# toandaominh1997/EfficientDet.Pytorch

Hardware: AMD Instinct MI355X
Metric: images/sec EfficientDet-D0 512px fwd+bwd (higher is better)
Workload: dtype f32_hf16x3_bwd_bf16x3

## Files before the change

### efficientdet/pytorch_amd/_lib.py

```python
import ctypes as C
import os

import torch

HERE = os.path.dirname(os.path.abspath(__file__))
LIB_PATH = os.environ.get('EFFDET_HIP_LIB') or os.path.join(os.path.dirname(os.path.abspath(__file__)), 'libeffdet_hip.so')
MAX_SEG = 5
MAX_CONV_SEG = 10
ABI_VERSION = 11
F32, BF16, F32_BF16X3, F32_SPLIT = 0, 1, 2, 3
F32_HSPLIT = 4
ACT_NONE, ACT_RELU, ACT_SWISH, ACT_SIGMOID = 0, 1, 2, 3
RES_NONE, RES_ADD, RES_RELU_MASK, RES_SWISH_GRAD = 0, 1, 2, 3
TUNE_IGEMM_BIG, TUNE_IGEMM_BIG_MIN_M, TUNE_SPLIT_PERS, TUNE_IGEMM_KORD, TUNE_SPLIT_KORD = 0, 1, 2, 3, 4
TUNE_ROWSLAB = 5
TUNE_SHORT_TILE = 7

_ERR = {-1: 'EFFDET_EINVAL', -2: 'EFFDET_ELAUNCH', -3: 'EFFDET_EUNSUPPORTED'}


class Seg(C.Structure):
    _fields_ = [('H', C.c_int), ('W', C.c_int), ('Ho', C.c_int), ('Wo', C.c_int),
                ('in_off', C.c_longlong), ('in_bstride', C.c_longlong),
                ('out_off', C.c_longlong), ('out_bstride', C.c_longlong)]


class ConvDesc(C.Structure):
    _fields_ = [('x', C.c_void_p), ('w', C.c_void_p), ('y', C.c_void_p), ('z', C.c_void_p), ('res', C.c_void_p),
                ('scale', C.c_void_p), ('shift', C.c_void_p), ('rowscale', C.c_void_p),
                ('bc_scale', C.c_void_p), ('bc_shift', C.c_void_p),
                ('dtype', C.c_int), ('out_f32', C.c_int),
# ... 78 lines not shown

class QualityLoss(C.Structure):
    _fields_ = [('kind', C.c_int), ('beta', C.c_float), ('alpha', C.c_float), ('gamma', C.c_float)]


TAL_MAX_TOPK = 16


class Tal(C.Structure):
    _fields_ = [('topk', C.c_int), ('alpha', C.c_float), ('beta', C.c_float), ('aligned_target', C.c_int)]


class ConvPlanInfo(C.Structure):
    _fields_ = [(n, C.c_int) for n in ('id', 'form', 'persistent', 'tile_m', 'tile_n', 'stages', 'threads', 'mtiles', 'ntiles', 'grid',
                                       'ksteps', 'kord', 'lds_bytes', 'm32')] + [('reserved', C.c_int * 2)]


class WgradPlanInfo(C.Structure):
    _fields_ = [(n, C.c_int) for n in ('path', 'splits', 'nfast', 'mchunk', 'ntiles', 'jtiles', 'stage_pixels', 'allr', 'thin_ns', 'gate',
                                       'nseg')] + [('first', C.c_int * MAX_SEG), ('count', C.c_int * MAX_SEG), ('reserved', C.c_int * 3)]


WBF_MAX_VIEWS, WBF_MAX_IN = 8, 4096


class Wbf(C.Structure):
    _fields_ = [(n, C.c_void_p * WBF_MAX_VIEWS) for n in ('score', 'label', 'boxes', 'count')] + \
               [('A', C.c_longlong * WBF_MAX_VIEWS)] + [(n, C.c_float * WBF_MAX_VIEWS) for n in ('weight', 'width', 'mul')] + \
               [('flip', C.c_int * WBF_MAX_VIEWS)] + [(n, C.c_int) for n in ('V', 'B', 'top_n', 'conf_type')] + \
               [('iou_thr', C.c_float), ('skip_thr', C.c_float)] + \
# ... 206 lines not shown
WGRAD_PAIR_SIGNATURES = {
    'effdet_conv2d_wgrad_pair': 'i:pppqps',
}
OPT_GROUPS_SIGNATURES = {
    'effdet_opt_step_groups': 'i:iippppppppppiiipppfiipps',
}
GATE_OPERAND_SIGNATURES = {
    'effdet_conv2d_gated': 'i:ppis',
    'effdet_conv2d_gated_plan_info': 'i:ppip',
    'effdet_conv2d_wgrad_gated': 'i:ppipqs',
    'effdet_conv2d_wgrad_gated_kernel': 'i:ppi',
}
WGRAD_PLAN_SIGNATURES = {
    'effdet_conv2d_wgrad_plan_info': 'i:pp',
}
RESAMPLE_SIGNATURES = {
    'effdet_resample_images': 'i:ps',
}
SLICES_SIGNATURES = {
    'effdet_slice_images': 'i:ps',
    'effdet_slice_merge_workspace_bytes': 'q:iii',
    'effdet_slice_merge': 'i:ppqs',
}
OP_POINT_SIGNATURES = {
    'effdet_op_curves_workspace_bytes': 'q:q',
    'effdet_op_curves': 'i:ppqpipipqppppppps',
    'effdet_confusion_match': 'i:ppppiiiifdps',
}
OP_MAX_THRESHOLDS = 4096
TRACK_SIGNATURES = {
# ... 23 lines not shown
        if not os.path.exists(LIB_PATH):
            raise RuntimeError(
                'libeffdet_hip.so is missing (%s). Build it with `python -m efficientdet.pytorch_amd.build` '
                '(or __graft_entry__.build()). There is no CPU fallback for this path.' % LIB_PATH)
        cand = C.CDLL(LIB_PATH)
        got = int(cand.effdet_abi_version()) if hasattr(cand, 'effdet_abi_version') else 0
        if got != ABI_VERSION:
            raise RuntimeError('%s has ABI generation %d, this binding needs %d: rebuild it (`python -m efficientdet.pytorch_amd.build`)'
                               % (LIB_PATH, got, ABI_VERSION))
        _lib = cand
        for name, sig in list(SIGNATURES.items()) + list(ADDED_SIGNATURES.items()) + list(EMA_SIGNATURES.items()) + \
                list(PLAN_SIGNATURES.items()) + list(LIVE_SIGNATURES.items()) + list(BOX_LOSS_SIGNATURES.items()) + \
                list(LOSS_OPTS_SIGNATURES.items()) + list(ATSS_SIGNATURES.items()) + list(CONV_PLAN_SIGNATURES.items()) + \
                list(WBF_SIGNATURES.items()) + list(NEEDED_SIGNATURES.items()) + list(MOSAIC_SIGNATURES.items()) + \
                list(WGRAD_PAIR_SIGNATURES.items()) + list(OPT_GROUPS_SIGNATURES.items()) + list(GATE_OPERAND_SIGNATURES.items()) + \
                list(WGRAD_PLAN_SIGNATURES.items()) + list(AFFINE_SIGNATURES.items()) + list(RESAMPLE_SIGNATURES.items()) + \
                list(UNIT_LISTS_SIGNATURES.items()) + list(SLICES_SIGNATURES.items()) + list(QUALITY_LOSS_SIGNATURES.items()) + \
                list(TAL_SIGNATURES.items()) + list(OP_POINT_SIGNATURES.items()) + list(TRACK_SIGNATURES.items()) + \
                list(ASSIGN_SIGNATURES.items()):
            f = getattr(_lib, name, None)
            if f is not None:
                f.restype, f.argtypes = _CTYPE[sig[0]], [_CTYPE[c] for c in sig[2:]]
    return _lib


def require(*names):
    L = lib()
    missing = [n for n in names if not hasattr(L, n)]
    if missing:
        raise RuntimeError('%s does not export %s: it predates this binding, rebuild it (`python -m efficientdet.pytorch_amd.build`)'
                           % (LIB_PATH, ', '.join(missing)))
# ... 28 lines not shown
```

### efficientdet/pytorch_amd/csrc/common.h

```cpp
#pragma once
#include <hip/hip_runtime.h>
#include <stdint.h>
#include "../../../include/effdet_hip.h"

typedef uint16_t bf16_t;
typedef float f32x4 __attribute__((ext_vector_type(4)));
typedef __bf16 bf16x8 __attribute__((ext_vector_type(8)));

#define EFFDET_CHECK_LAUNCH()                                 \
  do {                                                        \
    hipError_t e_ = hipGetLastError();                        \
    if (e_ != hipSuccess) return EFFDET_ELAUNCH;              \
  } while (0)

#define EFFDET_SET_MAX_LDS(kernel, bytes)                                                                           \
  do {                                                                                                              \
    static unsigned long long done_ = 0ull;                                                                         \
    int dev_ = 0;                                                                                                   \
    (void)hipGetDevice(&dev_);                                                                                      \
    const unsigned long long bit_ = 1ull << (dev_ & 63);                                                            \
    if (!(done_ & bit_)) {                                                                                          \
      (void)hipFuncSetAttribute((const void*)(kernel), hipFuncAttributeMaxDynamicSharedMemorySize, (int)(bytes));  \
      done_ |= bit_;                                                                                                \
    }                                                                                                               \
// ... 184 lines not shown
  return f32x4{__uint_as_float(v[0]), __uint_as_float(v[1]), __uint_as_float(v[2]), __uint_as_float(v[3])};
}
typedef unsigned u32x2_t __attribute__((ext_vector_type(2)));
template <> __device__ __forceinline__ f32x4 srd_load4<bf16_t>(__amdgpu_buffer_rsrc_t r, unsigned byte_off) {
  const u32x2_t u = __builtin_amdgcn_raw_buffer_load_b64(r, (int)byte_off, 0, 0);
  return f32x4{__uint_as_float(u[0] << 16), __uint_as_float(u[0] & 0xffff0000u), __uint_as_float(u[1] << 16),
               __uint_as_float(u[1] & 0xffff0000u)};
}

__device__ __forceinline__ int xcd_remap(int bid, int nwg) {
  const int q = nwg >> 3, r = nwg & 7;
  const int xcd = bid & 7, idx = bid >> 3;
  const int base = (xcd < r) ? xcd * (q + 1) : r * (q + 1) + (xcd - r) * q;
  return base + idx;
}
```

### efficientdet/pytorch_amd/csrc/conv_igemm.hip

```cpp
#include "common.h"
#include "../../../include/effdet_live_tiles.h"
#include "../../../include/effdet_needed_tiles.h"
#include "../../../include/effdet_unit_lists.h"
#include "../../../include/effdet_conv_plan.h"
#include "../../../include/effdet_gate_operand.h"
#include <stdlib.h>

#ifndef EFFDET_IGEMM_BIG_DEFAULT
#define EFFDET_IGEMM_BIG_DEFAULT 1
#endif

namespace {

struct SegD {
  int H, W, Ho, Wo, M, tile_start;
  long long in_off, in_bs, out_off, out_bs;
  unsigned x_bytes;
  long long w_off;
  long long sh_off;
};

struct ConvK {
  const void* x; const void* w; void* y; void* z; const void* res;
  const float* scale; const float* shift; const float* rowscale;
// ... 1205 lines not shown
}

struct ConvPlan {
  int id;
  ConvK k;
  int (*launch)(const ConvPlan&, hipStream_t);
  unsigned grid;
  size_t lds;
  int pw_G, pw_NPS, pw_ppw;
  int form, pers;
  int tile_m, tile_n, stages, threads, m32;
  int ksteps;
  int gate;
};

static int g_tuning[EFFDET_TUNE_COUNT] = {-1, 16384, -1, 1, -1, -1, 0 , 1};
static bool rowslab_on() {
  if (g_tuning[EFFDET_TUNE_ROWSLAB] < 0) g_tuning[EFFDET_TUNE_ROWSLAB] = getenv("EFFDET_ROWSLAB") ? atoi(getenv("EFFDET_ROWSLAB")) : 1;
  return g_tuning[EFFDET_TUNE_ROWSLAB] != 0;
}

template <typename T, int BN, int WAVES_N, int NWAVES, int SPLIT, int NS, int M32, int GATE, int BM>
int launch_igemm(const ConvPlan& c, hipStream_t st) {
  if (c.lds > 48 * 1024) EFFDET_SET_MAX_LDS((conv_igemm_kernel<T, BN, WAVES_N, NWAVES, SPLIT, NS, M32, GATE, BM>), c.lds);
  hipLaunchKernelGGL((conv_igemm_kernel<T, BN, WAVES_N, NWAVES, SPLIT, NS, M32, GATE, BM>), dim3(c.grid), dim3(NWAVES * 64), c.lds, st, c.k);
  EFFDET_CHECK_LAUNCH();
  return EFFDET_OK;
}
template <typename T, int BN, int WAVES_N, int NWAVES, int SPLIT = 0, int NS = 2, int M32 = 0, int GATE = 0, int BM = BM128>
int use_igemm(ConvPlan& c, int id) {
  if constexpr (BM != BM128) {
// ... 103 lines not shown
    }
    if (bt == 0) return use_igemm<T, 128, 2, 8, SPLIT, 4, 0, GATE>(c, id);
    if (bt == 1) return use_igemm<T, 64, 1, 4, SPLIT, 4, 0, GATE>(c, id);
  }
  switch (bt) {
    case 0: return use_igemm<T, 128, 2, 8, SPLIT, 2, 0, GATE>(c, id);
    case 1: return use_igemm<T, 64, 1, 4, SPLIT, 2, 0, GATE>(c, id);
    case 2: return use_igemm<T, 32, 1, 4, SPLIT, 2, 0, GATE>(c, id);
    default: return use_igemm<T, 16, 1, 4, SPLIT, 2, 0, GATE>(c, id);
  }
}

}

extern "C" int effdet_tuning_set(int key, int value) {
  if (key < 0 || key >= EFFDET_TUNE_COUNT || key == EFFDET_TUNE_ROWSLAB + 1) return EFFDET_EINVAL;
  (void)big_variant();
  const int old = g_tuning[key];
  g_tuning[key] = value;
  return old;
}

static int plan_conv(const effdet_conv_t* p, ConvPlan& c, const float* a_gate = nullptr, int a_act = EFFDET_ACT_NONE) {
  ConvK& k = c.k;
  c.gate = 0;
  if (!p || !p->x || !p->w || !p->y) return EFFDET_EINVAL;
  if (p->nseg < 1 || p->nseg > EFFDET_MAX_CONV_SEG) return EFFDET_EINVAL;
  if (p->dtype != EFFDET_F32 && p->dtype != EFFDET_BF16 && p->dtype != EFFDET_F32_BF16X3 && p->dtype != EFFDET_F32_SPLIT && p->dtype != EFFDET_F32_HSPLIT) return EFFDET_EINVAL;
  const int ce = p->dtype == EFFDET_BF16 ? 8 : 4;
  if (p->Cin % ce || p->ldx % ce || p->KH < 1 || p->KW < 1 || p->stride < 1) return EFFDET_EUNSUPPORTED;
  if (p->res_mode != EFFDET_RES_NONE && !p->res) return EFFDET_EINVAL;
  const bool hfmt = p->dtype == EFFDET_F32_HSPLIT;
  const bool splitfmt = p->dtype == EFFDET_F32_SPLIT || hfmt;
  if (hfmt && (p->res_mode != EFFDET_RES_NONE || p->scale || p->bc_scale || p->rowscale || p->w_image_stride || (p->KH * p->KW * p->Cin) % 32)) return EFFDET_EUNSUPPORTED;
  if (splitfmt) {
    if (p->Cin % 32 || p->ldx % 32 || p->z) return EFFDET_EUNSUPPORTED;
// ... 224 lines not shown
```

### efficientdet/pytorch_amd/csrc/conv_wgrad.hip

```cpp
#include "common.h"
#include "../../../include/effdet_gate_operand.h"
#include "../../../include/effdet_live_tiles.h"
#include "../../../include/effdet_wgrad_pair.h"
#include "../../../include/effdet_wgrad_plan.h"
#include <stdlib.h>

#ifndef EFFDET_WGRAD_TR_WAVES
#define EFFDET_WGRAD_TR_WAVES 8
#endif

namespace {

struct WSeg {
  int H, W, Ho, Wo, M, split_start;
  long long in_off, in_bs, out_off, out_bs;
  unsigned x_bytes, dz_bytes;
  int step0;
};
struct WgradK {
  const void* x; const void* dz; float* dw; float* dbias; float* slab;
  float* dbp;
  int Cin, Cout, KW, stride, pad_t, pad_l;
  int ldx, lddz;
  int B;
  int Kc, cpt;
  int K;
  int mchunk;
  int nseg, ntiles, jtiles, vec_a;
  const unsigned char* live32;
  const float* a_gate;
  int gate_hw;
  WSeg seg[EFFDET_MAX_SEG];
};

template <typename T> struct WMma;
template <> struct WMma<bf16_t> {
  static __device__ __forceinline__ void run(const uint4& a, const uint4& b, f32x4& c) {
    c = __builtin_amdgcn_mfma_f32_16x16x32_bf16(__builtin_bit_cast(bf16x8, a), __builtin_bit_cast(bf16x8, b), c, 0, 0, 0);
  }
  static __device__ __forceinline__ uint4 ones() { return make_uint4(0x3f803f80u, 0x3f803f80u, 0x3f803f80u, 0x3f803f80u); }
};
template <> struct WMma<float> {
  static __device__ __forceinline__ void run(const uint4& a, const uint4& b, f32x4& c) {
// ... 582 lines not shown
  const int prob = idx < nf ? q.first : q.first ^ 1;
  const int l = idx < nf ? f0 + idx : eighth((int)gridDim.x, xcd) - f0 + (idx - nf);
  int split, tile;
  if (LIVEB && prob == 1) { tile = l / q.splits[1]; split = q.splits[1] - 1 - (l - tile * q.splits[1]); }
  else { split = l / tiles; tile = l - split * tiles; }
  const int nt = tile % q.k.ntiles, jt = tile / q.k.ntiles;
  int si = 0;
#pragma unroll
  for (int s = 1; s < EFFDET_MAX_SEG; ++s)
    if (s < q.nseg[prob] && split >= q.seg[prob][s].split_start) si = s;
  const WSeg sg = q.seg[prob][si];
  if (LIVEB && prob == 1) wgrad_split_block<ALLR, 1>(q.k, sg, q.x[1], q.dz[1], q.slab[1], q.dbp[1], q.live32, nt, jt, split);
  else wgrad_split_block<ALLR, 0>(q.k, sg, q.x[prob], q.dz[prob], q.slab[prob], q.dbp[prob], nullptr, nt, jt, split);
}

template <int NW, int X3 = 0, int GATE = 0>
__global__ __launch_bounds__(NW * 64, (GATE && X3) ? 2 : 1) void conv_wgrad_f32dma_kernel(const WgradK p) {
  constexpr int WJ = NW / 2;
  constexpr int WTJ = 128 / WJ, JB = WTJ / 16;
  constexpr int BKM = 32;
  constexpr unsigned OPB = 16384, BUFB = 2 * OPB;
  constexpr int PPW = 16 / NW;

  extern __shared__ __attribute__((aligned(16))) uint4 smem[];
  const int tid = threadIdx.x, lane = tid & 63;
  const int wave = __builtin_amdgcn_readfirstlane(tid >> 6);
  const int wn0 = (wave / WJ) * 64, wj0 = (wave % WJ) * WTJ;
  const int logical = xcd_remap(blockIdx.x, gridDim.x);
  const int nt = logical % p.ntiles, jt = (logical / p.ntiles) % p.jtiles, split = logical / (p.ntiles * p.jtiles);
  int si = 0;
#pragma unroll
  for (int s = 1; s < EFFDET_MAX_SEG; ++s)
    if (s < p.nseg && split >= p.seg[s].split_start) si = s;
  const WSeg sg = p.seg[si];
  const int m_begin = (split - sg.split_start) * p.mchunk;
  const int m_end = min(sg.M, m_begin + p.mchunk);
  const int nsteps = (m_end - m_begin + BKM - 1) / BKM;
// ... 58 lines not shown
  float gb[JB];
  if constexpr (GATE) {
    const float* grow = p.a_gate + (long long)(m_begin / p.gate_hw) * p.K;
#pragma unroll
    for (int b = 0; b < JB; ++b) { const int j = jt * 128 + wj0 + JB * c15 + b; gb[b] = j < p.K ? grow[j] : 0.f; }
  }
  auto gate1 = [&](float v, int b) -> float {
    if constexpr (GATE == 2) v = swishf_(v);
    v *= gb[b];
    asm volatile("" : "+v"(v));
    return v;
  };

  if (nsteps > 0) {
    stage(0);
    if constexpr (X3) {
      typedef float f32x2l __attribute__((ext_vector_type(2)));
      auto split8 = [](const float (&v)[8], uint4& hi, uint4& lo) {
        unsigned h[4], l[4];
#pragma unroll
        for (int i = 0; i < 4; ++i) {
          h[i] = pack2bf(v[2 * i], v[2 * i + 1]);
          l[i] = pack2bf(v[2 * i] - __uint_as_float(h[i] << 16), v[2 * i + 1] - __uint_as_float(h[i] & 0xffff0000u));
        }
        hi = make_uint4(h[0], h[1], h[2], h[3]); lo = make_uint4(l[0], l[1], l[2], l[3]);
      };
      auto mm = [](const uint4& a, const uint4& b, f32x4& c) {
        c = __builtin_amdgcn_mfma_f32_16x16x32_bf16(__builtin_bit_cast(bf16x8, a), __builtin_bit_cast(bf16x8, b), c, 0, 0, 0);
      };
      const uint4 ones = make_uint4(0x3f803f80u, 0x3f803f80u, 0x3f803f80u, 0x3f803f80u);
      uint4 ah[4], al[4], bh[JB], bl[JB];
      bool have = false;
      auto mma_stage = [&]() {
#pragma unroll
        for (int t = 0; t < 3; ++t)
#pragma unroll
          for (int a = 0; a < 4; ++a)
#pragma unroll
            for (int b = 0; b < JB; ++b) mm(t == 0 ? al[a] : ah[a], t == 1 ? bl[b] : bh[b], acc[a][b]);
        if (want_bias) {
#pragma unroll
          for (int a = 0; a < 4; ++a) { mm(al[a], ones, bsum[a]); mm(ah[a], ones, bsum[a]); }
        }
      };
      for (int kt = 0; kt < nsteps; ++kt) {
        const unsigned cur = (unsigned)(kt & 1) * BUFB;
        dma_wait_all();
        __syncthreads();
        if (kt + 1 < nsteps) stage((kt & 1) ^ 1);
        f32x4 ra[8]; float rb[8][JB];
#pragma unroll
        for (int e = 0; e < 8; ++e) {
          ra[e] = *(const f32x4 __attribute__((address_space(3)))*)(size_t)(a_addr + cur + (unsigned)e * 2048u);
          if constexpr (JB == 4) {
            const f32x4 t = *(const f32x4 __attribute__((address_space(3)))*)(size_t)(b_addr + cur + (unsigned)e * 2048u);
#pragma unroll
            for (int b = 0; b < JB; ++b) rb[e][b] = t[b];
          } else {
            const f32x2l t = *(const f32x2l __attribute__((address_space(3)))*)(size_t)(b_addr + cur + (unsigned)e * 2048u);
            rb[e][0] = t[0]; rb[e][1] = t[1];
          }
        }
        __builtin_amdgcn_sched_barrier(0);
        if (have) mma_stage();
// ... 6 lines not shown
#pragma unroll
        for (int a = 0; a < 4; ++a) {
          const float v[8] = {ra[0][a], ra[1][a], ra[2][a], ra[3][a], ra[4][a], ra[5][a], ra[6][a], ra[7][a]};
          split8(v, ah[a], al[a]);
        }
#pragma unroll
        for (int b = 0; b < JB; ++b) {
          const float v[8] = {rb[0][b], rb[1][b], rb[2][b], rb[3][b], rb[4][b], rb[5][b], rb[6][b], rb[7][b]};
          split8(v, bh[b], bl[b]);
        }
        have = true;
      }
      mma_stage();
    } else {
      for (int kt = 0; kt < nsteps; ++kt) {
        const unsigned cur = (unsigned)(kt & 1) * BUFB;
        dma_wait_all();
        __syncthreads();
        if (kt + 1 < nsteps) stage((kt & 1) ^ 1);
        auto lda = [&](int ks) -> f32x4 { return *(const f32x4 __attribute__((address_space(3)))*)(size_t)(a_addr + cur + (unsigned)ks * 2048u); };
        auto ldb = [&](int ks) -> f32x4 {
          if constexpr (JB == 4) return *(const f32x4 __attribute__((address_space(3)))*)(size_t)(b_addr + cur + (unsigned)ks * 2048u);
          else {
            typedef float f32x2l __attribute__((ext_vector_type(2)));
            const f32x2l t = *(const f32x2l __attribute__((address_space(3)))*)(size_t)(b_addr + cur + (unsigned)ks * 2048u);
            return f32x4{t[0], t[1], 0.f, 0.f};
          }
        };
        f32x4 av = lda(0), bv = ldb(0);
        if constexpr (GATE) {
  #pragma unroll
          for (int b = 0; b < JB; ++b) bv[b] = gate1(bv[b], b);
        }
  #pragma unroll
// ... 32 lines not shown
          else { dst[0] = acc[a][0][reg]; dst[1] = acc[a][1][reg]; }
        } else {
#pragma unroll
          for (int b = 0; b < JB; ++b) if (j0 + b < p.K) dst[b] = acc[a][b][reg];
        }
        if (want_bias && c15 == 0) p.dbp[(long long)split * p.Cout + nn] = bsum[a][reg];
      }
    }
  } else {
    for (int i = tid; i < 128 * 128; i += NW * 64) {
      const int nn = nt * 128 + i / 128, j = jt * 128 + (i & 127);
      if (nn < p.Cout && j < p.K) slab[(long long)nn * p.K + j] = 0.f;
    }
    if (p.dbp && jt == 0 && tid < 128 && nt * 128 + tid < p.Cout) p.dbp[(long long)split * p.Cout + nt * 128 + tid] = 0.f;
  }
}

template <int NTA, int NTB, bool STEM = false, int GATE = 0>
__global__ __launch_bounds__(256) void conv_wgrad_thin_kernel(const WgradK p, int P, int pps, int NS) {
  static_assert(!GATE || !STEM, "the operand gate covers the pointwise form");
  extern __shared__ __attribute__((aligned(16))) uint4 smem[];
  const int tid = threadIdx.x, lane = tid & 63;
  const int wave = __builtin_amdgcn_readfirstlane(tid >> 6);
  const int split = blockIdx.x;
  const WSeg sg = p.seg[0];
  const int m_begin = split * p.mchunk, m_end = min(sg.M, m_begin + p.mchunk);
  const int Cin = STEM ? p.K : p.Cin, Cout = p.Cout;
  const unsigned xrow = (unsigned)Cin * 4u, zrow = (unsigned)Cout * 4u;
  const unsigned xstage = (unsigned)P * xrow, zstage = (unsigned)P * zrow;
  const int HoWo = sg.Ho * sg.Wo;
// ... 162 lines not shown
    s2 += part[(long long)(k + 2) * Cout + c]; s3 += part[(long long)(k + 3) * Cout + c];
  }
  for (; k < splits; ++k) s0 += part[(long long)k * Cout + c];
  dbias[c] += (s0 + s1) + (s2 + s3);
}

}

namespace {
int plan(const effdet_wgrad_t* p, WgradK& k, int& splits, int tile = 128) {
  if (!p || p->nseg < 1 || p->nseg > EFFDET_MAX_SEG) return EFFDET_EINVAL;
  if (p->dtype != EFFDET_F32 && p->dtype != EFFDET_BF16) return EFFDET_EINVAL;
  const int ce = p->dtype == EFFDET_F32 ? 4 : 8;
  if (p->Cin % ce || p->ldx % ce) return EFFDET_EUNSUPPORTED;
  k.x = p->x; k.dz = p->dz; k.dw = p->dw; k.dbias = p->dbias; k.slab = nullptr; k.dbp = nullptr; k.live32 = nullptr;
  k.Cin = p->Cin; k.Cout = p->Cout; k.KW = p->KW; k.stride = p->stride; k.pad_t = p->pad_t; k.pad_l = p->pad_l;
  k.ldx = p->ldx; k.lddz = p->lddz; k.B = p->B;
  k.cpt = p->Cin / ce; k.Kc = p->KH * p->KW * k.cpt; k.K = p->KH * p->KW * p->Cin;
  k.nseg = p->nseg;
  k.ntiles = (p->Cout + tile - 1) / tile; k.jtiles = (k.K + tile - 1) / tile;
  k.vec_a = (p->lddz % ce == 0) && (((p->Cout + ce - 1) / ce * ce) <= p->lddz) ? 1 : 0;
  const int bkm = 8 * ce;
  long long Mtot = 0;
  for (int s = 0; s < p->nseg; ++s) Mtot += (long long)p->B * p->seg[s].Ho * p->seg[s].Wo;
  const long long tiles = (long long)k.ntiles * k.jtiles;
  auto chunk_for = [&](long long sc) {
    long long mc = (Mtot + sc - 1) / sc;
    if (mc < 8LL * bkm) mc = 8LL * bkm;
    return (mc + bkm - 1) / bkm * bkm;
  };
// ... 104 lines not shown
  effdet_wgrad_t d;
  bool x3, split;
  int cout;
  int path;
  WgradK k;
  WgradK ks;
  int splits, nfast;
  int first[EFFDET_MAX_SEG], count[EFFDET_MAX_SEG];
  int P, NS, pps;
  WgradLaunch launch;
  WgradLaunch launch_live;
  WgradLaunch launch_rest;
  int gate;
  size_t lds;
  int allr;
  long long slab_floats;
  long long workspace_bytes;
};

template <auto Kernel, int THREADS, bool THIN = false, typename K = WgradK>
void launcher(const WgradPlan& w, const K& k, unsigned blocks, hipStream_t st) {
  EFFDET_SET_MAX_LDS(Kernel, w.lds);
  if constexpr (THIN) hipLaunchKernelGGL(Kernel, dim3(blocks), dim3(THREADS), w.lds, st, k, w.P, w.pps, w.NS);
  else hipLaunchKernelGGL(Kernel, dim3(blocks), dim3(THREADS), w.lds, st, k);
}
const WgradLaunch split_launch[2][2] = {
  {launcher<conv_wgrad_split_kernel<0, 0>, 512>, launcher<conv_wgrad_split_kernel<0, 1>, 512>},
  {launcher<conv_wgrad_split_kernel<1, 0>, 512>, launcher<conv_wgrad_split_kernel<1, 1>, 512>}};
void (*const pair_launch[2][2])(const WgradPlan&, const WgradPairK&, unsigned, hipStream_t) = {
  {launcher<conv_wgrad_pair_kernel<0, 0>, 512, false, WgradPairK>, launcher<conv_wgrad_pair_kernel<0, 1>, 512, false, WgradPairK>},
  {launcher<conv_wgrad_pair_kernel<1, 0>, 512, false, WgradPairK>, launcher<conv_wgrad_pair_kernel<1, 1>, 512, false, WgradPairK>}};
const WgradLaunch f32dma_launch[2][3] = {
  {launcher<conv_wgrad_f32dma_kernel<F32_NW, 0, 0>, F32_NW * 64>, launcher<conv_wgrad_f32dma_kernel<F32_NW, 0, 1>, F32_NW * 64>,
   launcher<conv_wgrad_f32dma_kernel<F32_NW, 0, 2>, F32_NW * 64>},
  {launcher<conv_wgrad_f32dma_kernel<X3_NW, 1, 0>, X3_NW * 64>, launcher<conv_wgrad_f32dma_kernel<X3_NW, 1, 1>, X3_NW * 64>,
   launcher<conv_wgrad_f32dma_kernel<X3_NW, 1, 2>, X3_NW * 64>}};
const WgradLaunch tr_launch = launcher<conv_wgrad_tr_kernel<TR_NW>, TR_NW * 64>;
const WgradLaunch rest_launch[2] = {launcher<conv_wgrad_kernel<float>, 256>, launcher<conv_wgrad_kernel<bf16_t>, 256>};
template <int NTA, int NTB, bool STEM = false, int GATE = 0>
constexpr WgradLaunch launch_thin = launcher<conv_wgrad_thin_kernel<NTA, NTB, STEM, GATE>, 256, true>;
#define THIN_(a, b) {a, b, {launch_thin<a, b>, launch_thin<a, b, false, 1>, launch_thin<a, b, false, 2>}}
const struct { int nta, ntb; WgradLaunch launch[3]; } thin_shapes[] = {
  THIN_(1, 2), THIN_(6, 1), THIN_(2, 6), THIN_(9, 2), THIN_(2, 9), THIN_(3, 9), THIN_(1, 1), THIN_(2, 1), THIN_(1, 3), THIN_(2, 2)};
#undef THIN_
WgradLaunch thin_launch(int nta, int ntb, int gate = 0) {
  for (const auto& t : thin_shapes) if (t.nta == nta && t.ntb == ntb) return t.launch[gate];
  return nullptr;
}
int thin_eligible(const effdet_wgrad_t* p, bool splitfmt) {
  static const int on = getenv("EFFDET_WGRAD_THIN") ? atoi(getenv("EFFDET_WGRAD_THIN")) : 1;
  if (!on || splitfmt || !p || p->dtype != EFFDET_F32 || p->nseg != 1) return 0;
// ... 6 lines not shown
    if (2 * (g.Ho - 1) - p->pad_t >= g.H || 2 * (g.Wo - 1) - p->pad_l >= g.W) return 0;
    return 2;
  }
  if (p->KH != 1 || p->KW != 1 || p->stride != 1 || p->pad_t || p->pad_l) return 0;
  if (g.Ho != g.H || g.Wo != g.W || p->ldx != p->Cin || (p->Cin & 3)) return 0;
  if (g.in_bstride != (long long)g.H * g.W * p->ldx) return 0;
  if ((g.in_off & 3) || p->Cin + p->Cout > 192) return 0;
  return thin_launch((p->Cout + 15) / 16, (p->Cin + 15) / 16) ? 1 : 0;
}

int plan_wgrad(const effdet_wgrad_t* p, WgradPlan& w, const float* a_gate = nullptr, int a_act = EFFDET_ACT_NONE) {
  if (!p) return EFFDET_EINVAL;
  if (a_gate && a_act != EFFDET_ACT_NONE && a_act != EFFDET_ACT_SWISH) return EFFDET_EINVAL;
  w.gate = a_gate ? (a_act == EFFDET_ACT_SWISH ? 2 : 1) : 0;
  w.launch = w.launch_live = w.launch_rest = nullptr;
  effdet_wgrad_t& q = w.d;
  q = *p; w.cout = q.Cout; w.x3 = w.split = false;
  if (q.dtype == EFFDET_F32_BF16X3) { q.dtype = EFFDET_F32; w.x3 = true; }
  else if (q.dtype == EFFDET_F32_SPLIT) {
    w.split = true; q.dtype = EFFDET_BF16;
    if (q.Cin % 32 || q.ldx % 32 || q.lddz % 32 || q.Cout > q.lddz || q.nseg < 1 || q.nseg > EFFDET_MAX_SEG) return EFFDET_EINVAL;
    q.Cin *= 2; q.ldx *= 2; q.Cout = 2 * q.lddz; q.lddz *= 2;
    for (int s = 0; s < q.nseg; ++s) { q.seg[s].in_off *= 2; q.seg[s].in_bstride *= 2; q.seg[s].out_off *= 2; q.seg[s].out_bstride *= 2; }
  }
  const int thin = thin_eligible(&q, w.split);
  WgradK& k = w.k;
  const int rc = plan(&q, k, w.splits, w.split || thin ? 256 : 128);
  if (rc != EFFDET_OK) return rc;
  k.a_gate = a_gate; k.gate_hw = 1;
  if (a_gate) {
// ... 47 lines not shown
  } else {
    w.path = WG_TILED;
    w.ks = k;
    int nf = 0, ns = 0;
    for (int s = 0; s < q.nseg; ++s) {
      WSeg d = w.ks.seg[s];
      if (fast[s]) { d.split_start = w.first[s]; flatten(d); k.seg[nf++] = d; }
      else { d.split_start = w.first[s] - sf; w.ks.seg[ns++] = d; }
    }
    for (int s = nf; s < EFFDET_MAX_SEG; ++s) { k.seg[s] = k.seg[0]; k.seg[s].split_start = 0x7fffffff; }
    for (int s = ns; s < EFFDET_MAX_SEG; ++s) { w.ks.seg[s] = w.ks.seg[0]; w.ks.seg[s].split_start = 0x7fffffff; }
    k.nseg = nf; w.ks.nseg = ns;
    w.lds = (size_t)4 * 128 * 8 * sizeof(uint4);
    if (a_gate && ns) return EFFDET_EUNSUPPORTED;
    if (nf) w.launch = q.dtype == EFFDET_F32 ? f32dma_launch[w.x3][w.gate] : tr_launch;
    if (ns) w.launch_rest = rest_launch[q.dtype == EFFDET_BF16];
  }
  w.slab_floats = (long long)w.cout * k.K;
  w.workspace_bytes = (long long)w.splits * (w.slab_floats + w.cout) * (long long)sizeof(float);
  return EFFDET_OK;
}

int reduce_slabs(const effdet_wgrad_t* p, const WgradPlan& w, const float* slab, const float* dbp, hipStream_t st) {
  if (!p->dw) return EFFDET_OK;
  const long long n = w.slab_floats;
  long long g = (n / 4 + 255) / 256; if (g < 1) g = 1; if (g > 4096) g = 4096;
  hipLaunchKernelGGL(wgrad_reduce_kernel, dim3((unsigned)g), dim3(256), 0, st, slab, p->dw, n, w.splits);
  EFFDET_CHECK_LAUNCH();
  if (p->dbias) {
    hipLaunchKernelGGL(wgrad_bias_reduce_kernel, dim3((unsigned)((w.cout + 255) / 256)), dim3(256), 0, st, dbp, p->dbias, w.cout, w.splits);
// ... 28 lines not shown
  return w.splits;
}

extern "C" int effdet_conv2d_wgrad_plan_info(const effdet_wgrad_t* p, effdet_wgrad_plan_info_t* info) {
  if (!p || !info) return EFFDET_EINVAL;
  WgradPlan w;
  const int rc = plan_wgrad(p, w);
  if (rc != EFFDET_OK) return rc;
  const bool thin = w.path == WG_THIN || w.path == WG_STEM;
  effdet_wgrad_plan_info_t o = {};
  o.path = w.path; o.splits = w.splits; o.nfast = w.nfast; o.mchunk = w.k.mchunk;
  o.ntiles = thin ? 1 : w.k.ntiles; o.jtiles = thin ? 1 : w.k.jtiles;
  o.stage_pixels = thin ? w.P : (w.path == WG_SPLIT || w.d.dtype == EFFDET_F32) ? 32 : 64;
  o.allr = w.path == WG_SPLIT ? w.allr : 0; o.thin_ns = thin ? w.NS : 0; o.gate = w.gate; o.nseg = p->nseg;
  for (int s = 0; s < p->nseg; ++s) { o.first[s] = w.first[s]; o.count[s] = w.count[s]; }
  *info = o;
  return w.path;
}

static int wgrad_launch(const effdet_wgrad_t* p, void* workspace, long long workspace_bytes, const unsigned char* live32,
                        effdet_stream_t stream, const float* a_gate = nullptr, int a_act = EFFDET_ACT_NONE) {
  if (!p || !p->x || !p->dz || !workspace) return EFFDET_EINVAL;
  WgradPlan w;
  const int rc = plan_wgrad(p, w, a_gate, a_act);
  if (rc != EFFDET_OK) return rc;
  if (a_gate && live32) return EFFDET_EUNSUPPORTED;
  if (workspace_bytes < w.workspace_bytes) return EFFDET_EINVAL;
  if (live32 && w.path != WG_SPLIT) return EFFDET_EUNSUPPORTED;
  if (live32 && w.k.mchunk % 32) return EFFDET_EINVAL;
  hipStream_t st = (hipStream_t)stream;
// ... 82 lines not shown
```

### efficientdet/pytorch_amd/ops.py

```python
import ctypes as C
import os
import threading

import numpy as np
import torch

from . import _lib as L
from ._lib import (ACT_NONE, ACT_RELU, ACT_SIGMOID, ACT_SWISH, RES_ADD, RES_NONE,
                   RES_RELU_MASK, RES_SWISH_GRAD)


class LaunchProfile:

    def __init__(self):
        self.records = []

    def summary(self):
        torch.cuda.synchronize()
        out = {}
        for name, flops, e0, e1, _, nbytes in self.records:
            d = out.setdefault(name, {'launches': 0, 'flops': 0.0, 'ms': 0.0, 'bytes': 0.0})
            d['launches'] += 1; d['flops'] += flops; d['ms'] += e0.elapsed_time(e1); d['bytes'] += nbytes
        return out

# ... 506 lines not shown


def conv2d_wgrad_kernel_id(x, dz, *, Cin, Cout, KH, KW, stride=1, pad_t=0, pad_l=0, split=False, image_splits=False, a_gate=None,
                           a_act=ACT_NONE):
    d = _wgrad_desc([x], [dz], None, None, Cin, Cout, KH, KW, stride, pad_t, pad_l, True, split, image_splits)
    return _wgrad_gated_kernel(d, a_gate, a_act) if a_gate is not None else int(L.lib().effdet_conv2d_wgrad_kernel(C.byref(d)))


def conv2d_wgrad_plan_info(xs, dzs, dw=None, dbias=None, *, Cin, Cout, KH, KW, stride=1, pad_t=0, pad_l=0, want_bias=True, split=False,
                           image_splits=False, **_launch_only):
    if isinstance(xs, Map):
        xs, dzs = [xs], [dzs]
    return _wgrad_plan(_wgrad_desc(xs, dzs, dw, dbias, Cin, Cout, KH, KW, stride, pad_t, pad_l, want_bias, split, image_splits))


def _wgrad_plan(d, refused=None):
    info = L.WgradPlanInfo()
    rc = int(L.require('effdet_conv2d_wgrad_plan_info').effdet_conv2d_wgrad_plan_info(C.byref(d), C.byref(info)))
    if rc < 0:
        if refused is not None:
            raise RuntimeError(refused)
        L.check(rc, 'effdet_conv2d_wgrad_plan_info')
    out = {n: int(getattr(info, n)) for n, _ in L.WgradPlanInfo._fields_ if n not in ('first', 'count', 'reserved', 'nseg')}
    out['path'], out['allr'] = L.WGRAD_PATHS[out['path']], bool(out['allr'])
    out['first'], out['count'] = list(info.first[:info.nseg]), list(info.count[:info.nseg])
    return out


def _wgrad_views(ws, splits, Cout, taps, Cin, bias, first=0, count=None):
    n, r = Cout * taps * Cin, slice(first, splits if count is None else first + count)
# ... 2047 lines not shown
```

### include/effdet_hip.h

```cpp
#ifndef EFFDET_HIP_H
#define EFFDET_HIP_H
#ifdef __cplusplus
extern "C" {
#endif

typedef void* effdet_stream_t;

enum { EFFDET_OK = 0, EFFDET_EINVAL = -1, EFFDET_ELAUNCH = -2, EFFDET_EUNSUPPORTED = -3 };
enum { EFFDET_F32 = 0, EFFDET_BF16 = 1,
       EFFDET_F32_BF16X3 = 2,
       EFFDET_F32_SPLIT = 3,
       EFFDET_F32_HSPLIT = 4 };
enum { EFFDET_ACT_NONE = 0, EFFDET_ACT_RELU = 1, EFFDET_ACT_SWISH = 2, EFFDET_ACT_SIGMOID = 3 };
enum { EFFDET_RES_NONE = 0, EFFDET_RES_ADD = 1, EFFDET_RES_RELU_MASK = 2, EFFDET_RES_SWISH_GRAD = 3 };

#define EFFDET_MAX_SEG 5
#define EFFDET_MAX_CONV_SEG 10

typedef struct {
  int H, W, Ho, Wo;
  long long in_off, in_bstride, out_off, out_bstride;
} effdet_seg_t;

typedef struct {
// ... 12 lines not shown
  int* range_flag;
  const void* seg_w[EFFDET_MAX_CONV_SEG];
  const float* seg_shift[EFFDET_MAX_CONV_SEG];
} effdet_conv_t;
int effdet_conv2d(const effdet_conv_t* p, effdet_stream_t stream);
int effdet_scale_pack_weight(const float* w, const float* gate, void* out, int dtype, int B, int Cout, int Cin, effdet_stream_t stream);

int effdet_conv2d_kernel(const effdet_conv_t* p);

enum { EFFDET_TUNE_IGEMM_BIG = 0, EFFDET_TUNE_IGEMM_BIG_MIN_M = 1,
       EFFDET_TUNE_SPLIT_PERS = 2 ,
       EFFDET_TUNE_IGEMM_KORD = 3 ,
       EFFDET_TUNE_SPLIT_KORD = 4 ,
       EFFDET_TUNE_ROWSLAB = 5 ,
       EFFDET_TUNE_SHORT_TILE = 7 ,
       EFFDET_TUNE_COUNT = 8 };
int effdet_tuning_set(int key, int value);

typedef struct {
  const void* x; const void* dz; float* dw; float* dbias;
  int dtype;
  int B, Cin, Cout, KH, KW, stride, pad_t, pad_l;
  int ldx, lddz;
  int nseg;
  int image_splits;
  effdet_seg_t seg[EFFDET_MAX_SEG];
} effdet_wgrad_t;
long long effdet_conv2d_wgrad_workspace_bytes(const effdet_wgrad_t* p);
int effdet_conv2d_wgrad_splits(const effdet_wgrad_t* p);
int effdet_conv2d_wgrad_seg_slabs(const effdet_wgrad_t* p, int* first, int* count);
int effdet_conv2d_wgrad_kernel(const effdet_wgrad_t* p);
// ... 295 lines not shown
```

Baseline: 1449.

## Add deep-ring and half-width tile variants to the x3 f32 DMA wgrad kernel

Generalises the f32 DMA weight-gradient kernel with a configurable number of LDS stages (ring buffer with partial vmcnt waits) and a wave layout that uses all waves along one dimension for a last output tile with at most 64 live channels. The planner picks a 4-stage ring for small grids and the half-width layout for narrow trailing tiles on the bf16x3 path, under a new tuning key that defaults to on. The aim is better latency hiding when there are few workgroups and less wasted MMA work on partially filled Cout tiles. The cost is more LDS per block, which can lower occupancy, plus more kernel instantiations.

```diff
diff --git a/efficientdet/pytorch_amd/_lib.py b/efficientdet/pytorch_amd/_lib.py
--- a/efficientdet/pytorch_amd/_lib.py
+++ b/efficientdet/pytorch_amd/_lib.py
@@ -15,6 +15,7 @@
 TUNE_IGEMM_BIG, TUNE_IGEMM_BIG_MIN_M, TUNE_SPLIT_PERS, TUNE_IGEMM_KORD, TUNE_SPLIT_KORD = 0, 1, 2, 3, 4
 TUNE_ROWSLAB = 5
 TUNE_SHORT_TILE = 7
+TUNE_WGRAD_NARROW = 9
 
 _ERR = {-1: 'EFFDET_EINVAL', -2: 'EFFDET_ELAUNCH', -3: 'EFFDET_EUNSUPPORTED'}
 
@@ -123,6 +124,10 @@
 class ConvPlanInfo(C.Structure):
     _fields_ = [(n, C.c_int) for n in ('id', 'form', 'persistent', 'tile_m', 'tile_n', 'stages', 'threads', 'mtiles', 'ntiles', 'grid',
                                        'ksteps', 'kord', 'lds_bytes', 'm32')] + [('reserved', C.c_int * 2)]
+
+
+class WgradNarrowInfo(C.Structure):
+    _fields_ = [(n, C.c_int) for n in ('ring', 'stages', 'half_tile', 'lds_bytes', 'grid', 'ntiles', 'gate')] + [('reserved', C.c_int * 5)]
 
 
 class WgradPlanInfo(C.Structure):
@@ -359,6 +364,9 @@
 WGRAD_PLAN_SIGNATURES = {
     'effdet_conv2d_wgrad_plan_info': 'i:pp',
 }
+WGRAD_NARROW_SIGNATURES = {
+    'effdet_conv2d_wgrad_narrow_info': 'i:ppip',
+}
 RESAMPLE_SIGNATURES = {
     'effdet_resample_images': 'i:ps',
 }
@@ -412,7 +420,7 @@
                 list(LOSS_OPTS_SIGNATURES.items()) + list(ATSS_SIGNATURES.items()) + list(CONV_PLAN_SIGNATURES.items()) + \
                 list(WBF_SIGNATURES.items()) + list(NEEDED_SIGNATURES.items()) + list(MOSAIC_SIGNATURES.items()) + \
                 list(WGRAD_PAIR_SIGNATURES.items()) + list(OPT_GROUPS_SIGNATURES.items()) + list(GATE_OPERAND_SIGNATURES.items()) + \
-                list(WGRAD_PLAN_SIGNATURES.items()) + list(AFFINE_SIGNATURES.items()) + list(RESAMPLE_SIGNATURES.items()) + \
+                list(WGRAD_PLAN_SIGNATURES.items()) + list(WGRAD_NARROW_SIGNATURES.items()) + list(AFFINE_SIGNATURES.items()) + list(RESAMPLE_SIGNATURES.items()) + \
                 list(UNIT_LISTS_SIGNATURES.items()) + list(SLICES_SIGNATURES.items()) + list(QUALITY_LOSS_SIGNATURES.items()) + \
                 list(TAL_SIGNATURES.items()) + list(OP_POINT_SIGNATURES.items()) + list(TRACK_SIGNATURES.items()) + \
                 list(ASSIGN_SIGNATURES.items()):
diff --git a/efficientdet/pytorch_amd/csrc/common.h b/efficientdet/pytorch_amd/csrc/common.h
--- a/efficientdet/pytorch_amd/csrc/common.h
+++ b/efficientdet/pytorch_amd/csrc/common.h
@@ -222,3 +222,5 @@
   const int base = (xcd < r) ? xcd * (q + 1) : r * (q + 1) + (xcd - r) * q;
   return base + idx;
 }
+
+int effdet_tune_wgrad_narrow();
diff --git a/efficientdet/pytorch_amd/csrc/conv_igemm.hip b/efficientdet/pytorch_amd/csrc/conv_igemm.hip
--- a/efficientdet/pytorch_amd/csrc/conv_igemm.hip
+++ b/efficientdet/pytorch_amd/csrc/conv_igemm.hip
@@ -1243,7 +1243,7 @@
   int gate;
 };
 
-static int g_tuning[EFFDET_TUNE_COUNT] = {-1, 16384, -1, 1, -1, -1, 0 , 1};
+static int g_tuning[EFFDET_TUNE_COUNT] = {-1, 16384, -1, 1, -1, -1, 0 , 1, 0 , 1};
 static bool rowslab_on() {
   if (g_tuning[EFFDET_TUNE_ROWSLAB] < 0) g_tuning[EFFDET_TUNE_ROWSLAB] = getenv("EFFDET_ROWSLAB") ? atoi(getenv("EFFDET_ROWSLAB")) : 1;
   return g_tuning[EFFDET_TUNE_ROWSLAB] != 0;
@@ -1377,12 +1377,14 @@
 }
 
 extern "C" int effdet_tuning_set(int key, int value) {
-  if (key < 0 || key >= EFFDET_TUNE_COUNT || key == EFFDET_TUNE_ROWSLAB + 1) return EFFDET_EINVAL;
+  if (key < 0 || key >= EFFDET_TUNE_COUNT || key == EFFDET_TUNE_ROWSLAB + 1 || key == EFFDET_TUNE_SHORT_TILE + 1) return EFFDET_EINVAL;
   (void)big_variant();
   const int old = g_tuning[key];
   g_tuning[key] = value;
   return old;
 }
+
+int effdet_tune_wgrad_narrow() { return g_tuning[EFFDET_TUNE_WGRAD_NARROW]; }
 
 static int plan_conv(const effdet_conv_t* p, ConvPlan& c, const float* a_gate = nullptr, int a_act = EFFDET_ACT_NONE) {
   ConvK& k = c.k;
diff --git a/efficientdet/pytorch_amd/csrc/conv_wgrad.hip b/efficientdet/pytorch_amd/csrc/conv_wgrad.hip
--- a/efficientdet/pytorch_amd/csrc/conv_wgrad.hip
+++ b/efficientdet/pytorch_amd/csrc/conv_wgrad.hip
@@ -3,6 +3,7 @@
 #include "../../../include/effdet_live_tiles.h"
 #include "../../../include/effdet_wgrad_pair.h"
 #include "../../../include/effdet_wgrad_plan.h"
+#include "../../../include/effdet_wgrad_narrow.h"
 #include <stdlib.h>
 
 #ifndef EFFDET_WGRAD_TR_WAVES
@@ -27,6 +28,7 @@
   int K;
   int mchunk;
   int nseg, ntiles, jtiles, vec_a;
+  int narrow;
   const unsigned char* live32;
   const float* a_gate;
   int gate_hw;
@@ -639,13 +641,23 @@
   else wgrad_split_block<ALLR, 0>(q.k, sg, q.x[prob], q.dz[prob], q.slab[prob], q.dbp[prob], nullptr, nt, jt, split);
 }
 
-template <int NW, int X3 = 0, int GATE = 0>
-__global__ __launch_bounds__(NW * 64, (GATE && X3) ? 2 : 1) void conv_wgrad_f32dma_kernel(const WgradK p) {
-  constexpr int WJ = NW / 2;
+template <int PPS, int A>
+__device__ __forceinline__ void wgrad_ring_wait(int ahead) {
+  if constexpr (A == 0) { (void)ahead; dma_wait_all(); }
+  else {
+    if (ahead >= A) asm volatile("s_waitcnt vmcnt(%0)" :: "n"(A * PPS) : "memory");
+    else wgrad_ring_wait<PPS, A - 1>(ahead);
+  }
+}
+template <int NW, int X3, int GATE, int WN, int NS>
+__device__ __forceinline__ void wgrad_f32dma_body(const WgradK& p) {
+  constexpr int WJ = NW / WN;
   constexpr int WTJ = 128 / WJ, JB = WTJ / 16;
   constexpr int BKM = 32;
   constexpr unsigned OPB = 16384, BUFB = 2 * OPB;
   constexpr int PPW = 16 / NW;
+  constexpr int PPS = 2 * PPW;
+  static_assert(NS >= 2 && !(NS & (NS - 1)) && (NS - 2) * PPS <= 63 && (JB == 4 || JB == 2), "a count s_waitcnt vmcnt can hold; a 16- or 8-byte B read");
 
   extern __shared__ __attribute__((aligned(16))) uint4 smem[];
   const int tid = threadIdx.x, lane = tid & 63;
@@ -734,6 +746,9 @@
 
   if (nsteps > 0) {
     stage(0);
+#pragma unroll
+    for (int s = 1; s < NS - 1; ++s)
+      if (s < nsteps) stage(s);
     if constexpr (X3) {
       typedef float f32x2l __attribute__((ext_vector_type(2)));
       auto split8 = [](const float (&v)[8], uint4& hi, uint4& lo) {
@@ -764,10 +779,11 @@
         }
       };
       for (int kt = 0; kt < nsteps; ++kt) {
-        const unsigned cur = (unsigned)(kt & 1) * BUFB;
-        dma_wait_all();
+        const unsigned cur = (unsigned)(kt & (NS - 1)) * BUFB;
+        wgrad_ring_wait<PPS, NS - 2>(nsteps - 1 - kt);
         __syncthreads();
-        if (kt + 1 < nsteps) stage((kt & 1) ^ 1);
+        if constexpr (NS == 2) { if (kt + 1 < nsteps) stage((kt & 1) ^ 1); }
+        else if (kt + NS - 1 < nsteps) stage((kt + NS - 1) & (NS - 1));
         f32x4 ra[8]; float rb[8][JB];
 #pragma unroll
         for (int e = 0; e < 8; ++e) {
@@ -804,10 +820,11 @@
       mma_stage();
     } else {
       for (int kt = 0; kt < nsteps; ++kt) {
-        const unsigned cur = (unsigned)(kt & 1) * BUFB;
-        dma_wait_all();
+        const unsigned cur = (unsigned)(kt & (NS - 1)) * BUFB;
+        wgrad_ring_wait<PPS, NS - 2>(nsteps - 1 - kt);
         __syncthreads();
-        if (kt + 1 < nsteps) stage((kt & 1) ^ 1);
+        if constexpr (NS == 2) { if (kt + 1 < nsteps) stage((kt & 1) ^ 1); }
+        else if (kt + NS - 1 < nsteps) stage((kt + NS - 1) & (NS - 1));
         auto lda = [&](int ks) -> f32x4 { return *(const f32x4 __attribute__((address_space(3)))*)(size_t)(a_addr + cur + (unsigned)ks * 2048u); };
         auto ldb = [&](int ks) -> f32x4 {
           if constexpr (JB == 4) return *(const f32x4 __attribute__((address_space(3)))*)(size_t)(b_addr + cur + (unsigned)ks * 2048u);
@@ -870,6 +887,16 @@
     }
     if (p.dbp && jt == 0 && tid < 128 && nt * 128 + tid < p.Cout) p.dbp[(long long)split * p.Cout + nt * 128 + tid] = 0.f;
   }
+}
+template <int NW, int X3 = 0, int GATE = 0>
+__global__ __launch_bounds__(NW * 64, (GATE && X3) ? 2 : 1) void conv_wgrad_f32dma_kernel(const WgradK p) {
+  wgrad_f32dma_body<NW, X3, GATE, 2, 2>(p);
+}
+template <int GATE, int NS>
+__global__ __launch_bounds__(256, GATE ? 2 : 1) void conv_wgrad_f32dma_ring_kernel(const WgradK p) {
+  const int nt = xcd_remap(blockIdx.x, gridDim.x) % p.ntiles;
+  if (p.narrow && p.Cout - nt * 128 <= 64) wgrad_f32dma_body<4, 1, GATE, 1, NS>(p);
+  else wgrad_f32dma_body<4, 1, GATE, 2, NS>(p);
 }
 
 template <int NTA, int NTB, bool STEM = false, int GATE = 0>
@@ -1062,6 +1089,7 @@
   const int ce = p->dtype == EFFDET_F32 ? 4 : 8;
   if (p->Cin % ce || p->ldx % ce) return EFFDET_EUNSUPPORTED;
   k.x = p->x; k.dz = p->dz; k.dw = p->dw; k.dbias = p->dbias; k.slab = nullptr; k.dbp = nullptr; k.live32 = nullptr;
+  k.narrow = 0;
   k.Cin = p->Cin; k.Cout = p->Cout; k.KW = p->KW; k.stride = p->stride; k.pad_t = p->pad_t; k.pad_l = p->pad_l;
   k.ldx = p->ldx; k.lddz = p->lddz; k.B = p->B;
   k.cpt = p->Cin / ce; k.Kc = p->KH * p->KW * k.cpt; k.K = p->KH * p->KW * p->Cin;
@@ -1196,6 +1224,7 @@
   int gate;
   size_t lds;
   int allr;
+  int stages, half_tile;
   long long slab_floats;
   long long workspace_bytes;
 };
@@ -1217,6 +1246,11 @@
    launcher<conv_wgrad_f32dma_kernel<F32_NW, 0, 2>, F32_NW * 64>},
   {launcher<conv_wgrad_f32dma_kernel<X3_NW, 1, 0>, X3_NW * 64>, launcher<conv_wgrad_f32dma_kernel<X3_NW, 1, 1>, X3_NW * 64>,
    launcher<conv_wgrad_f32dma_kernel<X3_NW, 1, 2>, X3_NW * 64>}};
+const WgradLaunch ring_launch[2][3] = {
+  {launcher<conv_wgrad_f32dma_ring_kernel<0, 2>, 256>, launcher<conv_wgrad_f32dma_ring_kernel<1, 2>, 256>, launcher<conv_wgrad_f32dma_ring_kernel<2, 2>, 256>},
+  {launcher<conv_wgrad_f32dma_ring_kernel<0, 4>, 256>, launcher<conv_wgrad_f32dma_ring_kernel<1, 4>, 256>, launcher<conv_wgrad_f32dma_ring_kernel<2, 4>, 256>}};
+constexpr int WGRAD_HALF_LIVE = 64;
+constexpr int WGRAD_DEEP_MAX_WG = 256;
 const WgradLaunch tr_launch = launcher<conv_wgrad_tr_kernel<TR_NW>, TR_NW * 64>;
 const WgradLaunch rest_launch[2] = {launcher<conv_wgrad_kernel<float>, 256>, launcher<conv_wgrad_kernel<bf16_t>, 256>};
 template <int NTA, int NTB, bool STEM = false, int GATE = 0>
@@ -1253,6 +1287,7 @@
   if (a_gate && a_act != EFFDET_ACT_NONE && a_act != EFFDET_ACT_SWISH) return EFFDET_EINVAL;
   w.gate = a_gate ? (a_act == EFFDET_ACT_SWISH ? 2 : 1) : 0;
   w.launch = w.launch_live = w.launch_rest = nullptr;
+  w.stages = 2; w.half_tile = -1;
   effdet_wgrad_t& q = w.d;
   q = *p; w.cout = q.Cout; w.x3 = w.split = false;
   if (q.dtype == EFFDET_F32_BF16X3) { q.dtype = EFFDET_F32; w.x3 = true; }
@@ -1330,6 +1365,19 @@
     w.lds = (size_t)4 * 128 * 8 * sizeof(uint4);
     if (a_gate && ns) return EFFDET_EUNSUPPORTED;
     if (nf) w.launch = q.dtype == EFFDET_F32 ? f32dma_launch[w.x3][w.gate] : tr_launch;
+    if (nf && !ns && w.x3) {
+      const int tune = effdet_tune_wgrad_narrow();
+      const int live = w.cout - (k.ntiles - 1) * 128;
+      const bool half = (tune == 1 || tune == 2) && live <= WGRAD_HALF_LIVE;
+      const bool deep = (tune == 1 || tune == 3) && (long long)k.ntiles * k.jtiles * w.nfast <= WGRAD_DEEP_MAX_WG;
+      if (half || deep) {
+        k.narrow = half ? 1 : 0;
+        w.half_tile = half ? k.ntiles - 1 : -1;
+        w.stages = deep ? 4 : 2;
+        w.launch = ring_launch[deep ? 1 : 0][w.gate];
+        w.lds = (size_t)w.stages * 32768;
+      }
+    }
     if (ns) w.launch_rest = rest_launch[q.dtype == EFFDET_BF16];
   }
   w.slab_floats = (long long)w.cout * k.K;
@@ -1388,6 +1436,24 @@
   o.stage_pixels = thin ? w.P : (w.path == WG_SPLIT || w.d.dtype == EFFDET_F32) ? 32 : 64;
   o.allr = w.path == WG_SPLIT ? w.allr : 0; o.thin_ns = thin ? w.NS : 0; o.gate = w.gate; o.nseg = p->nseg;
   for (int s = 0; s < p->nseg; ++s) { o.first[s] = w.first[s]; o.count[s] = w.count[s]; }
+  *info = o;
+  return w.path;
+}
+
+extern "C" int effdet_conv2d_wgrad_narrow_info(const effdet_wgrad_t* p, const float* a_gate, int a_act, effdet_wgrad_narrow_info_t* info) {
+  if (!p || !info) return EFFDET_EINVAL;
+  WgradPlan w;
+  const int rc = plan_wgrad(p, w, a_gate, a_act);
+  if (rc != EFFDET_OK) return rc;
+  effdet_wgrad_narrow_info_t o = {};
+  const bool tiled = w.path == WG_TILED && w.launch;
+  o.ring = tiled && w.x3 && (w.stages != 2 || w.half_tile >= 0) ? 1 : 0;
+  o.stages = tiled || w.path == WG_SPLIT ? w.stages : 0;
+  o.half_tile = tiled ? w.half_tile : -1;
+  o.lds_bytes = (int)w.lds;
+  o.grid = (w.path == WG_TILED || w.path == WG_SPLIT ? w.k.ntiles * w.k.jtiles : 1) * w.nfast;
+  o.ntiles = w.path == WG_THIN || w.path == WG_STEM ? 1 : w.k.ntiles;
+  o.gate = w.gate;
   *info = o;
   return w.path;
 }
diff --git a/efficientdet/pytorch_amd/ops.py b/efficientdet/pytorch_amd/ops.py
--- a/efficientdet/pytorch_amd/ops.py
+++ b/efficientdet/pytorch_amd/ops.py
@@ -544,6 +544,21 @@
     return _wgrad_plan(_wgrad_desc(xs, dzs, dw, dbias, Cin, Cout, KH, KW, stride, pad_t, pad_l, want_bias, split, image_splits))
 
 
+def conv2d_wgrad_narrow_info(xs, dzs, dw=None, dbias=None, *, Cin, Cout, KH, KW, stride=1, pad_t=0, pad_l=0, want_bias=True, split=False,
+                             image_splits=False, a_gate=None, a_act=ACT_NONE, **_launch_only):
+    if isinstance(xs, Map):
+        xs, dzs = [xs], [dzs]
+    d = _wgrad_desc(xs, dzs, dw, dbias, Cin, Cout, KH, KW, stride, pad_t, pad_l, want_bias, split, image_splits)
+    info = L.WgradNarrowInfo()
+    rc = int(L.require('effdet_conv2d_wgrad_narrow_info').effdet_conv2d_wgrad_narrow_info(
+        C.byref(d), a_gate.data_ptr() if a_gate is not None else None, int(a_act), C.byref(info)))
+    if rc < 0:
+        L.check(rc, 'effdet_conv2d_wgrad_narrow_info')
+    out = {n: int(getattr(info, n)) for n, _ in L.WgradNarrowInfo._fields_ if n != 'reserved'}
+    out['path'], out['ring'] = L.WGRAD_PATHS[rc], bool(out['ring'])
+    return out
+
+
 def _wgrad_plan(d, refused=None):
     info = L.WgradPlanInfo()
     rc = int(L.require('effdet_conv2d_wgrad_plan_info').effdet_conv2d_wgrad_plan_info(C.byref(d), C.byref(info)))
diff --git a/include/effdet_hip.h b/include/effdet_hip.h
--- a/include/effdet_hip.h
+++ b/include/effdet_hip.h
@@ -50,7 +50,8 @@
        EFFDET_TUNE_SPLIT_KORD = 4 ,
        EFFDET_TUNE_ROWSLAB = 5 ,
        EFFDET_TUNE_SHORT_TILE = 7 ,
-       EFFDET_TUNE_COUNT = 8 };
+       EFFDET_TUNE_WGRAD_NARROW = 9 ,
+       EFFDET_TUNE_COUNT = 10 };
 int effdet_tuning_set(int key, int value);
 
 typedef struct {
diff --git a/include/effdet_wgrad_narrow.h b/include/effdet_wgrad_narrow.h
--- /dev/null
+++ b/include/effdet_wgrad_narrow.h
@@ -0,0 +1,19 @@
+#ifndef EFFDET_WGRAD_NARROW_H
+#define EFFDET_WGRAD_NARROW_H
+#include "effdet_hip.h"
+#ifdef __cplusplus
+extern "C" {
+#endif
+
+typedef struct effdet_wgrad_narrow_info_t {
+  int ring, stages, half_tile, lds_bytes;
+  int grid, ntiles, gate;
+  int reserved[5];
+} effdet_wgrad_narrow_info_t;
+
+int effdet_conv2d_wgrad_narrow_info(const effdet_wgrad_t* p, const float* a_gate, int a_act, effdet_wgrad_narrow_info_t* info);
+
+#ifdef __cplusplus
+}
+#endif
+#endif
```

New measurement: 1452, median of 3. About the same (+0.2%).
